# Autobot37/weatherforecastingtoolkit

Hardware: AMD Instinct MI355X
Metric: SEVIR 384x384 frames/sec (AE train step) (higher is better)
Workload: dtype f32; 1 GPU; experiments/ae_v2 conv AE (ae_64x8x8_lin.PosAwareAE_TF, img_size=384), 1x384x384 synthetic SEVIR frames, batch 32/GPU, fp32, fwd + L1 + bwd + AdamW + cosine-warmup LR; batch_per_gpu=32, global_batch=32, img_size=384, parallelism=dp1, params=215033281

## Files before the change

### include/wfae.h

```cpp
#ifndef WFAE_H
#define WFAE_H

#include <stddef.h>
#include <stdint.h>

#ifdef __cplusplus
extern "C" {
#endif

typedef void* wfae_stream_t;

typedef enum {
  WFAE_OK = 0,
  WFAE_ERR_BAD_SHAPE = -1,
  WFAE_ERR_NULL_POINTER = -2,
  WFAE_ERR_WORKSPACE = -3,
  WFAE_ERR_LAUNCH = -4,
  WFAE_ERR_UNSUPPORTED = -5
} wfae_status;

int wfae_version(void);
const char* wfae_last_error_string(void);
size_t wfae_workspace_bytes(int64_t max_weight_elems);

// ... 29 lines not shown
int wfae_c1r_stat_rows(int M, int K, int NB, int HW);
int wfae_c1r_fwd(const float* w, int64_t w_sm, int64_t w_sk, const float* x, const float* pro_scale, const float* pro_shift,
                 const float* res, float* y, int NB, int K, int M, int HW, double* stat_part, int64_t stat_capacity,
                 int* stat_rows, wfae_stream_t stream);
int wfae_c1r_bnred_supported(int M, int K, int HW);
int wfae_c1r_bnred(const float* w, int64_t w_sm, int64_t w_sk, const float* dt, const float* x, const float* bn_scale,
                   const float* bn_shift, const float* save_mean, const float* save_invstd, float* da, int NB, int K, int M, int HW,
                   double* part, int64_t part_capacity, int* part_rows, wfae_stream_t stream);
int wfae_bn_act_bwd_from_rows(const double* part, int rows, int C, float* dgamma, float* dbeta, int accumulate, void* ws,
                              size_t ws_bytes, wfae_stream_t stream);
int wfae_c1r_bndx(const float* w, int64_t w_sm, int64_t w_sk, const float* dt, const float* x, const float* gamma,
                  const float* bn_scale, const float* bn_shift, const float* save_mean, const float* save_invstd, const float* coef,
                  const float* res, float* dx, int NB, int K, int M, int HW, int training, wfae_stream_t stream);
int wfae_c1rb_supported(int M, int K, int HW);
int wfae_c1rb_stat_rows(int M, int K, int NB, int HW);
int wfae_c1rb_fwd(const float* w, int64_t w_sm, int64_t w_sk, const uint16_t* x, const float* pro_scale, const float* pro_shift,
                  const uint16_t* res, uint16_t* y, int NB, int K, int M, int HW, double* stat_part, int64_t stat_capacity,
                  int* stat_rows, wfae_stream_t stream);
int wfae_c1w_supported(int Cin, int Cout, int HW);
int wfae_c1w_bwd_weight(const float* dy, const float* x, const float* bn_scale, const float* bn_shift, float* dw, int NB, int Cin,
                        int Cout, int HW, int accumulate, void* ws, size_t ws_bytes, wfae_stream_t stream);
int wfae_c1w_bwd_weight_bf16(const uint16_t* dy, const uint16_t* x, const float* bn_scale, const float* bn_shift, float* dw, int NB,
                             int Cin, int Cout, int HW, int accumulate, void* ws, size_t ws_bytes, wfae_stream_t stream);
int wfae_set_c1wd(int on);
int wfae_get_c1wd(void);
int wfae_c1wd_supported(int C, int mid, int HW);
int wfae_c1wd_bwd(const float* dy, const float* t2, const float* bn_scale, const float* bn_shift, const float* w3, float* dw3,
                  float* da3, int NB, int C, int mid, int HW, int accumulate, void* ws, size_t ws_bytes, wfae_stream_t stream);
int wfae_set_c1ws(int on);
int wfae_get_c1ws(void);
int wfae_c1ws_supported(int C, int mid, int HW);
int wfae_c1ws_stat_rows(int C, int mid, int NB, int HW, size_t ws_bytes);
int wfae_c1ws_bwd(const float* x, const float* dt1, const float* bn_scale, const float* bn_shift, const float* save_mean,
                  const float* save_invstd, const float* w1, float* dw1, double* part, int64_t part_capacity, int* part_rows, int NB,
                  int C, int mid, int HW, int accumulate, void* ws, size_t ws_bytes, wfae_stream_t stream);
int wfae_linear_fwd(const float* x, const float* w, const float* bias, float* y, int B, int In,
                    int Out, void* ws, size_t ws_bytes, wfae_stream_t stream);
int wfae_linear_bwd_data(const float* dy, const float* w, float* dx, int B, int In, int Out,
                         wfae_stream_t stream);
int wfae_linear_bwd_weight(const float* dy, const float* x, float* dw, int B, int In, int Out,
                           int accumulate, wfae_stream_t stream);
int wfae_linear_bwd_data_splitk(const float* dy, const float* w, float* dx, int B, int In, int Out, void* ws,
                                size_t ws_bytes, wfae_stream_t stream);
int wfae_linear_bwd_weight_splitk(const float* dy, const float* x, float* dw, int B, int In, int Out, int accumulate,
                                  void* ws, size_t ws_bytes, wfae_stream_t stream);

int wfae_conv4x4s2_down(const float* hi, const float* w, float* lo, int NB, int Chi, int Clo,
                        int Hlo, int Wlo, wfae_stream_t stream);
int wfae_conv4x4s2_up(const float* lo, const float* w, float* hi, int NB, int Chi, int Clo, int Hlo,
                      int Wlo, void* ws, size_t ws_bytes, wfae_stream_t stream);
int wfae_conv4x4s2_wgrad(const float* lo, const float* hi, float* dw, int NB, int Chi, int Clo,
// ... 391 lines not shown
```

### weatherforecastingtoolkit_amd/csrc/c1w.hip

```cpp
#include "common.h"

using namespace wfae;

namespace {

typedef float f32x16 __attribute__((ext_vector_type(16)));
typedef __bf16 bf16x8 __attribute__((ext_vector_type(8)));
typedef unsigned u32x4 __attribute__((ext_vector_type(4)));
typedef unsigned u32x2 __attribute__((ext_vector_type(2)));

struct C1WP {
  const void* P;
  const void* Q;
  float* slab;
  const float* pro_scale;
  const float* pro_shift;
  int MP, MQ, HW;
  int cpi;
  int kc;
  int ptiles;
};

constexpr int WNT = 512, WBK = 32;

// ... 176 lines not shown
      __builtin_amdgcn_sched_barrier(0);
      read_frag(f0, cur ^ 1, 0);
      mfma_frag(f1);
      __builtin_amdgcn_sched_barrier(0);
    }
  }

  float* __restrict__ Cb = p.slab + (long)blockIdx.y * p.MP * p.MQ;
#pragma unroll
  for (int i = 0; i < TM; ++i)
#pragma unroll
    for (int j = 0; j < TN; ++j) {
      const int col = n0 + wn0 + 32 * j + r31;
#pragma unroll
      for (int q = 0; q < 16; ++q) {
        const int row = m0 + wm0 + 32 * i + (q & 3) + 8 * (q >> 2) + 4 * lh;
        if (row < p.MP && col < p.MQ) Cb[(long)row * p.MQ + col] = acc[i][j][q];
      }
    }
}

inline bool al16(const void* q) { return (reinterpret_cast<uintptr_t>(q) & 15) == 0; }

template <typename T, int PRO>
int launch_c1w(C1WP& p, int NB, hipStream_t st, const char* what) {
  const int tm = p.MP > 128 ? 2 : 1, tn = p.MQ > 64 ? 2 : 1;
  const int bm = 128 * tm, bn = 64 * tn;
  p.ptiles = cdiv(p.MP, bm);
  const int qtiles = cdiv(p.MQ, bn);
  const dim3 grid((unsigned)(p.ptiles * qtiles), (unsigned)(NB * p.cpi)), block(WNT);
  if (tm == 2 && tn == 2) hipLaunchKernelGGL((c1w_kernel<T, 2, 2, PRO>), grid, block, 0, st, p);
  else if (tm == 2) hipLaunchKernelGGL((c1w_kernel<T, 2, 1, PRO>), grid, block, 0, st, p);
  else if (tn == 2) hipLaunchKernelGGL((c1w_kernel<T, 1, 2, PRO>), grid, block, 0, st, p);
  else hipLaunchKernelGGL((c1w_kernel<T, 1, 1, PRO>), grid, block, 0, st, p);
  return check_launch(what);
}

inline bool c1w_shape_ok(int Cin, int Cout, int HW) {
  return HW % 32 == 0 && Cin % 32 == 0 && Cout % 32 == 0 && Cin >= 32 && Cout >= 32;
}

template <typename T>
int c1w_impl(const T* dy, const T* x, const float* bn_scale, const float* bn_shift, float* dw, int NB, int Cin, int Cout, int HW,
             int accumulate, void* ws, size_t ws_bytes, hipStream_t st, const char* what) {
  WFAE_REQUIRE(dy && x && dw && ws, WFAE_ERR_NULL_POINTER, "%s: null pointer", what);
  WFAE_REQUIRE(NB > 0 && Cin > 0 && Cout > 0 && HW > 0 && NB <= 65535, WFAE_ERR_BAD_SHAPE, "%s: bad shape", what);
  WFAE_REQUIRE(c1w_shape_ok(Cin, Cout, HW) && al16(dy) && al16(x), WFAE_ERR_UNSUPPORTED,
               "%s: needs HW %% 32 == 0, channel counts %% 32 == 0, 16-byte aligned tensors (Cin %d, Cout %d, HW %d)", what, Cin,
               Cout, HW);
  const bool x_is_p = Cin >= Cout;
  C1WP p = {};
  p.P = x_is_p ? (const void*)x : (const void*)dy;
  p.Q = x_is_p ? (const void*)dy : (const void*)x;
  p.MP = x_is_p ? Cin : Cout;
// ... 18 lines not shown

namespace wfae {

bool c1w_chunks(int MP, int MQ, int NB, int HW, size_t ws_bytes, int* cpi_out, int* kc_out) {
  const size_t slab = (size_t)MP * MQ * sizeof(float);
  const int tiles = cdiv(MP, MP > 128 ? 256 : 128) * cdiv(MQ, MQ > 64 ? 128 : 64);
  int cpi = cdiv(1024, (long)tiles * NB);
  const int max_cpi = HW / 256 > 0 ? HW / 256 : 1;
  if (cpi > max_cpi) cpi = max_cpi;
  if (cpi < 1) cpi = 1;
  while (cpi > 1 && (size_t)NB * cpi * slab > ws_bytes) --cpi;
  if ((size_t)NB * cpi * slab > ws_bytes) return false;
  *kc_out = cdiv(cdiv(HW, cpi), WBK) * WBK;
  *cpi_out = cdiv(HW, *kc_out);
  return true;
}

}

extern "C" {

int wfae_c1w_supported(int Cin, int Cout, int HW) { return c1w_shape_ok(Cin, Cout, HW) ? 1 : 0; }

int wfae_c1w_bwd_weight(const float* dy, const float* x, const float* bn_scale, const float* bn_shift, float* dw, int NB, int Cin,
                        int Cout, int HW, int accumulate, void* ws, size_t ws_bytes, wfae_stream_t stream) {
  WFAE_REQUIRE((bn_scale != nullptr) == (bn_shift != nullptr), WFAE_ERR_NULL_POINTER, "c1w_bwd_weight: scale / shift go together");
  return c1w_impl(dy, x, bn_scale, bn_shift, dw, NB, Cin, Cout, HW, accumulate, ws, ws_bytes, (hipStream_t)stream, "c1w_bwd_weight");
}

int wfae_c1w_bwd_weight_bf16(const uint16_t* dy, const uint16_t* x, const float* bn_scale, const float* bn_shift, float* dw, int NB,
                             int Cin, int Cout, int HW, int accumulate, void* ws, size_t ws_bytes, wfae_stream_t stream) {
  WFAE_REQUIRE((bn_scale != nullptr) == (bn_shift != nullptr), WFAE_ERR_NULL_POINTER, "c1w_bwd_weight_bf16: scale / shift go together");
  return c1w_impl(dy, x, bn_scale, bn_shift, dw, NB, Cin, Cout, HW, accumulate, ws, ws_bytes, (hipStream_t)stream,
                  "c1w_bwd_weight_bf16");
}

}
```

### weatherforecastingtoolkit_amd/csrc/c1wd.hip

```cpp
#include "common.h"
#include <atomic>
#include <stdlib.h>
#include <type_traits>

using namespace wfae;

namespace {

typedef float f32x4 __attribute__((ext_vector_type(4)));
typedef float f32x16 __attribute__((ext_vector_type(16)));
typedef __bf16 bf16x8 __attribute__((ext_vector_type(8)));
typedef short s16x4 __attribute__((ext_vector_type(4)));
typedef short s16x8 __attribute__((ext_vector_type(8)));
typedef unsigned u32x4 __attribute__((ext_vector_type(4)));
typedef unsigned u32x2 __attribute__((ext_vector_type(2)));

struct C1WDP {
  const float* dy;
  const float* t2;
  const float* w3;
  const float* pro_scale;
  const float* pro_shift;
  float* slab;
  float* da;
  int HW;
  int cpi;
  int kc;
};

constexpr int DNT = 512, DBK = 32;

__device__ __forceinline__ unsigned off_row(int r, int c) { return (unsigned)(r * 64 + ((c ^ ((r >> 2) & 3)) << 4)); }

__device__ __forceinline__ void split_pair(float a, float b, unsigned& h, unsigned& m, unsigned& l) {
  h = pack_bf16(a, b);
  const float ra = a - bf16_lo(h), rb = b - bf16_hi(h);
  m = pack_bf16(ra, rb);
  l = pack_bf16(ra - bf16_lo(m), rb - bf16_hi(m));
}

template <int C>
__global__ __launch_bounds__(DNT, C == 128 ? 4 : 2) void c1wd_kernel(C1WDP p) {
  constexpr int M = C / 4;
  constexpr int TM = C / 128;
  constexpr int WQ = M / 32;
  constexpr int NDW = 4 * WQ;
  constexpr bool BOTH = NDW == 8;
  constexpr int KCH = C / 32;
  constexpr int LPR = 8;
  constexpr int P_LD = C * LPR, Q_LD = M * LPR;
  constexpr int P_IT = P_LD / DNT;
  static_assert(P_LD % DNT == 0 && Q_LD <= DNT, "loader");
  constexpr int A_PLANE_B = C * 64, B_PLANE_B = M * 64;
  constexpr int A_STAGE_B = 3 * A_PLANE_B, STAGE_B = 3 * (A_PLANE_B + B_PLANE_B);
  __shared__ __attribute__((aligned(16))) unsigned char smem[2 * STAGE_B];
  const int t = threadIdx.x, lane = t & 63;
  const int wave = __builtin_amdgcn_readfirstlane(t >> 6);
  const int img = blockIdx.x / p.cpi, chunk = blockIdx.x - img * p.cpi;
  const int k_begin = chunk * p.kc;
  const int k_end = min(p.HW, k_begin + p.kc);
  const int nsteps = (k_end - k_begin) / DBK;
  const bool do_dw = BOTH || wave < NDW, do_da = BOTH || wave >= NDW;

  const float* Pb = p.dy + (long)img * C * p.HW + k_begin;
  const float* Qb = p.t2 + (long)img * M * p.HW + k_begin;
  const float* p_src[P_IT];
  unsigned p_dst[P_IT];
#pragma unroll
  for (int j = 0; j < P_IT; ++j) {
    const int idx = t + j * DNT, r = idx / LPR, e = idx % LPR;
    p_src[j] = Pb + (long)r * p.HW + e * 4;
    p_dst[j] = off_row(r, e >> 1) + (unsigned)((e & 1) * 8);
  }
  const bool q_on = Q_LD == DNT || t < Q_LD;
  const int q_r = q_on ? t / LPR : 0, q_e = t % LPR;
  const float* q_src = Qb + (long)q_r * p.HW + q_e * 4;
  const unsigned q_dst = off_row(q_r, q_e >> 1) + (unsigned)((q_e & 1) * 8);
  const float q_s = p.pro_scale[q_r], q_h = p.pro_shift[q_r];
  u32x4 rp[P_IT], rq;
  auto load_global = [&]() {
#pragma unroll
    for (int j = 0; j < P_IT; ++j) rp[j] = *reinterpret_cast<const u32x4*>(p_src[j]);
    if (q_on) rq = *reinterpret_cast<const u32x4*>(q_src);
  };
  auto advance = [&](bool more) {
#pragma unroll
    for (int j = 0; j < P_IT; ++j) p_src[j] += more ? DBK : 0;
    q_src += more ? DBK : 0;
  };
  auto put = [&](unsigned char* base, int plane_b, unsigned dst, u32x4 r, bool act, float s, float h) {
    const unsigned u0 = r[0], u1 = r[1], u2 = r[2], u3 = r[3];
    float v0 = __uint_as_float(u0), v1 = __uint_as_float(u1), v2 = __uint_as_float(u2), v3 = __uint_as_float(u3);
    if (act) {
      v0 = gelu_f(fmaf(v0, s, h)); v1 = gelu_f(fmaf(v1, s, h));
      v2 = gelu_f(fmaf(v2, s, h)); v3 = gelu_f(fmaf(v3, s, h));
    }
    unsigned h0, m0, l0, h1, m1, l1;
    split_pair(v0, v1, h0, m0, l0);
    split_pair(v2, v3, h1, m1, l1);
    *reinterpret_cast<u32x2*>(base + dst) = u32x2{h0, h1};
    *reinterpret_cast<u32x2*>(base + plane_b + dst) = u32x2{m0, m1};
    *reinterpret_cast<u32x2*>(base + 2 * plane_b + dst) = u32x2{l0, l1};
  };
  auto store_lds = [&](int buf) {
    unsigned char* s = smem + buf * STAGE_B;
#pragma unroll
    for (int j = 0; j < P_IT; ++j) put(s, A_PLANE_B, p_dst[j], rp[j], false, 0.f, 0.f);
    if (q_on) put(s + A_STAGE_B, B_PLANE_B, q_dst, rq, true, q_s, q_h);
  };

  const int wm0 = (BOTH ? (wave >> 1) : (wave & 3)) * (32 * TM), wn0 = BOTH ? (wave & 1) * 32 : 0;
  const int r31 = lane & 31, lh = lane >> 5;
  const unsigned a_rd = (unsigned)((wm0 + r31) * 64), b_rd = (unsigned)((wn0 + r31) * 64);
  const int a_x = (r31 >> 2) & 3;
  f32x16 acc[TM];
  struct Frag {
    bf16x8 a[TM][3], b[3];
  };
  auto read_frag = [&](Frag& f, int buf, int ks) {
    const unsigned char* s = smem + buf * STAGE_B;
    const unsigned a_c = (unsigned)(((2 * ks + lh) ^ a_x) << 4);
#pragma unroll
    for (int i = 0; i < TM; ++i)
#pragma unroll
      for (int pl = 0; pl < 3; ++pl)
        f.a[i][pl] = *reinterpret_cast<const bf16x8*>(s + pl * A_PLANE_B + a_rd + i * (32 * 64) + a_c);
#pragma unroll
    for (int pl = 0; pl < 3; ++pl) f.b[pl] = *reinterpret_cast<const bf16x8*>(s + A_STAGE_B + pl * B_PLANE_B + b_rd + a_c);
  };
  auto mfma_frag = [&](const Frag& f) {
#pragma unroll
// ... 15 lines not shown
  bf16x8 wa[KCH][3];
  auto load_weights = [&]() {
#pragma unroll
    for (int ch = 0; ch < KCH; ++ch) {
      const float* src = p.w3 + (long)(32 * ch + 8 * kg) * M + 16 * mt + n16;
      float v[8];
#pragma unroll
      for (int e = 0; e < 8; ++e) v[e] = src[e * M];
      u32x4 h, m, l;
#pragma unroll
      for (int e = 0; e < 4; ++e) {
        unsigned qh, qm, ql;
        split_pair(v[2 * e], v[2 * e + 1], qh, qm, ql);
        h[e] = qh; m[e] = qm; l[e] = ql;
      }
      wa[ch][0] = __builtin_bit_cast(bf16x8, h);
      wa[ch][1] = __builtin_bit_cast(bf16x8, m);
      wa[ch][2] = __builtin_bit_cast(bf16x8, l);
    }
  };
  unsigned tr_rd[2];
#pragma unroll
  for (int hf = 0; hf < 2; ++hf) tr_rd[hf] = off_row(8 * kg + 4 * hf + tq, 2 * pt + (tp >> 1)) + 8u * (unsigned)(tp & 1);
  float* const da_dst = p.da + ((long)img * M + 16 * mt + 4 * kg) * p.HW + k_begin + 16 * pt + n16;
  auto da_step = [&](int buf, int st) {
    const unsigned char* s = smem + buf * STAGE_B;
    constexpr int PA[6] = {2, 0, 1, 1, 0, 0}, PB[6] = {0, 2, 1, 0, 1, 0};
    f32x4 d = {0.f, 0.f, 0.f, 0.f};
#pragma unroll
    for (int ch = 0; ch < KCH; ++ch) {
      bf16x8 b[3];
#pragma unroll
      for (int pl = 0; pl < 3; ++pl) {
        s16x4 part[2];
#pragma unroll
        for (int hf = 0; hf < 2; ++hf)
          part[hf] = __builtin_amdgcn_ds_read_tr16_b64_v4i16(
              (s16x4 __attribute__((address_space(3)))*)(s + pl * A_PLANE_B + ch * (32 * 64) + tr_rd[hf]));
        b[pl] = __builtin_bit_cast(bf16x8, __builtin_shufflevector(part[0], part[1], 0, 1, 2, 3, 4, 5, 6, 7));
      }
#pragma unroll
      for (int pr = 0; pr < 6; ++pr) d = __builtin_amdgcn_mfma_f32_16x16x32_bf16(wa[ch][PA[pr]], b[PB[pr]], d, 0, 0, 0);
    }
    float* o = da_dst + 32 * st;
#pragma unroll
    for (int q = 0; q < 4; ++q) o[(long)q * p.HW] = d[q];
  };

  auto run = [&](auto dwc, auto dac) {
    constexpr bool DW = decltype(dwc)::value, DA = decltype(dac)::value;
    if constexpr (DW) {
#pragma unroll
      for (int i = 0; i < TM; ++i)
#pragma unroll
        for (int q = 0; q < 16; ++q) acc[i][q] = 0.f;
    }
    if constexpr (DA) load_weights();
    if (nsteps > 0) {
      Frag f0, f1;
      load_global();
      advance(nsteps > 1);
      store_lds(0);
      load_global();
      advance(nsteps > 2);
      __syncthreads();
      if constexpr (DW) read_frag(f0, 0, 0);
      for (int st = 0; st < nsteps; ++st) {
        const int cur = st & 1;
        if constexpr (DW) read_frag(f1, cur, 1);
        store_lds(cur ^ 1);
        load_global();
        advance(st + 3 < nsteps);
        if constexpr (DW) mfma_frag(f0);
        if constexpr (DA) da_step(cur, st);
        __builtin_amdgcn_sched_barrier(0);
        __syncthreads();
        __builtin_amdgcn_sched_barrier(0);
        if constexpr (DW) {
          read_frag(f0, cur ^ 1, 0);
          mfma_frag(f1);
        }
        __builtin_amdgcn_sched_barrier(0);
      }
    }
    if constexpr (DW) {
      float* __restrict__ Cb = p.slab + (long)blockIdx.x * C * M;
#pragma unroll
      for (int i = 0; i < TM; ++i)
#pragma unroll
        for (int q = 0; q < 16; ++q) {
          const int row = wm0 + 32 * i + (q & 3) + 8 * (q >> 2) + 4 * lh;
          Cb[(long)row * M + wn0 + r31] = acc[i][q];
        }
    }
  };
  if constexpr (BOTH) run(std::true_type{}, std::true_type{});
  else if (do_dw) run(std::true_type{}, std::false_type{});
  else run(std::false_type{}, std::true_type{});
}

std::atomic<int> g_c1wd{-1};
inline bool c1wd_on() {
  int v = g_c1wd.load(std::memory_order_relaxed);
  if (v < 0) {
    const char* e = getenv("WFAE_C1WD");
    v = (e && e[0] == '0') ? 0 : 1;
    g_c1wd.store(v, std::memory_order_relaxed);
  }
  return v == 1;
}

inline bool al16(const void* q) { return (reinterpret_cast<uintptr_t>(q) & 15) == 0; }

inline bool c1wd_shape_ok(int C, int mid, int HW) { return (C == 128 || C == 256) && mid * 4 == C && HW > 0 && HW % 64 == 0; }

}

extern "C" {

int wfae_set_c1wd(int on) {
  g_c1wd.store(on ? 1 : 0, std::memory_order_relaxed);
  return WFAE_OK;
}

int wfae_get_c1wd(void) { return c1wd_on() ? 1 : 0; }

int wfae_c1wd_supported(int C, int mid, int HW) {
  return (c1wd_on() && c1wd_shape_ok(C, mid, HW) && wfae::split_gemm_enabled()) ? 1 : 0;
}

int wfae_c1wd_bwd(const float* dy, const float* t2, const float* bn_scale, const float* bn_shift, const float* w3, float* dw3,
                  float* da3, int NB, int C, int mid, int HW, int accumulate, void* ws, size_t ws_bytes, wfae_stream_t stream) {
  WFAE_REQUIRE(dy && t2 && bn_scale && bn_shift && w3 && dw3 && da3 && ws, WFAE_ERR_NULL_POINTER, "c1wd_bwd: null pointer");
  WFAE_REQUIRE(NB > 0 && C > 0 && mid > 0 && HW > 0 && NB <= 65535 && (int64_t)NB * HW < (1ll << 31), WFAE_ERR_BAD_SHAPE,
               "c1wd_bwd: bad shape");
  WFAE_REQUIRE(c1wd_shape_ok(C, mid, HW), WFAE_ERR_UNSUPPORTED,
               "c1wd_bwd: serves C = 128 or 256 with mid = C / 4 and HW %% 64 == 0 (C %d, mid %d, HW %d)", C, mid, HW);
  WFAE_REQUIRE(c1wd_on() && wfae::split_gemm_enabled(), WFAE_ERR_UNSUPPORTED,
               "c1wd_bwd: needs fp32 precision with the split GEMMs on and wfae_set_c1wd(1)");
  WFAE_REQUIRE(al16(dy) && al16(t2), WFAE_ERR_UNSUPPORTED, "c1wd_bwd: dy and t2 must be 16-byte aligned");
  C1WDP p = {};
  p.dy = dy; p.t2 = t2; p.w3 = w3;
  p.pro_scale = bn_scale; p.pro_shift = bn_shift;
  p.slab = (float*)ws; p.da = da3;
  p.HW = HW;
  WFAE_REQUIRE(c1w_chunks(C, mid, NB, HW, ws_bytes, &p.cpi, &p.kc), WFAE_ERR_WORKSPACE, "c1wd_bwd: workspace %zu < %zu", ws_bytes,
               (size_t)NB * C * mid * sizeof(float));
  hipStream_t st = (hipStream_t)stream;
  const dim3 grid((unsigned)(NB * p.cpi)), block(DNT);
  if (C == 128) hipLaunchKernelGGL((c1wd_kernel<128>), grid, block, 0, st, p);
  else hipLaunchKernelGGL((c1wd_kernel<256>), grid, block, 0, st, p);
  const int rc = check_launch("c1wd_bwd");
  if (rc) return rc;
  return slab_reduce((const float*)ws, dw3, nullptr, (long)C * mid, mid, NB * p.cpi, accumulate, st, 0);
}

}
```

### weatherforecastingtoolkit_amd/functional.py

```python
from __future__ import annotations

import os

import torch
from torch.autograd import Function

from . import ops

BN_EPS = 1e-5


_overlap = False
_side = {}


STAT_FUSION = os.environ.get("WFAE_STAT_FUSION", "1") == "1"


FUSE_A1 = os.environ.get("WFAE_FUSE_A1", "1") == "1"
FUSE_A1_MAXC = 1 << 30
FUSE_A3 = os.environ.get("WFAE_FUSE_A3", "1") == "1"
FUSE_A3_MAXC = int(os.environ.get("WFAE_FUSE_A3_MAXC", "128"))
FUSE_A3_MAXC_C1R = max(FUSE_A3_MAXC, 256)

# ... 501 lines not shown
        t2 = _g3_fwd(a2, wg, groups)
        st3 = _bn_stats(t2, bn3, training)
        a3 = None if fused3 else ops.bn_act_fwd(t2, st3, 1)
        y, mod._out_stats = _c1(w3, W3p[0], False, *((t2, st3) if fused3 else (a3, None)), x, emit, r3)
        ctx.save_for_backward(x, _opt(a1), t1, a2, t2, _opt(a3), g1, w1, g2, wg, g3, w3,
                              st1.mean, st1.invstd, st1.scale, st1.shift,
                              st2.mean, st2.invstd, st2.scale, st2.shift,
                              st3.mean, st3.invstd, st3.scale, st3.shift,
                              _opt(W1p[1] if d1 == "c1b" else None), _opt(W3p[1] if d3 == "c1b" else None))
        ctx.training = training
        ctx.groups = groups
        ctx.betas = (b1, b2, b3)
        return y

    @staticmethod
    def backward(ctx, dy):
        (x, a1, t1, a2, t2, a3, g1, w1, g2, wg, g3, w3, *s) = ctx.saved_tensors
        st1, st2, st3 = _mk_stats(*s[0:4]), _mk_stats(*s[4:8]), _mk_stats(*s[8:12])
        W1t, W3t = s[12], s[13]
        tr = ctx.training
        dy = _c(dy)
        mid = w1.shape[0]
        dw3 = grad_buffer(w3)
        da3 = None
        if a3.numel() == 0:
            if ops.conv1x1_wd_route(dy.shape[1], mid, dy.shape[2] * dy.shape[3], _storage(dy)) == "c1wd":
                da3 = _on_main(lambda: ops.conv1x1_bwd_wd(dy, t2, st3, w3, dw3))
            if da3 is None:
                _wgrad(lambda: ops.conv1x1_bwd_weight_bnact(dy, t2, st3, dw3), dy, t2, st3.scale, st3.shift)
        else:
            _wgrad(lambda: ops.conv1x1_bwd_weight(dy, a3, dw3), dy, a3)
        dg3, db3 = grad_buffer(g3), grad_buffer(ctx.betas[2])
        if da3 is not None:
            dt2 = ops.bn_act_bwd(da3, t2, g3, st3, dg3, db3, None, 1, tr)
        else:
            dt2 = _dgrad_bn(dy, w3, W3t, t2, g3, st3, dg3, db3, None, tr)
        del da3
        dwg = grad_buffer(wg)
        _wgrad(lambda: _g3_wgrad(dt2, a2, dwg, ctx.groups), dt2, a2)
        da2 = _g3_dgrad(dt2, wg, mid, ctx.groups)
        del dt2
        dg2, db2 = grad_buffer(g2), grad_buffer(ctx.betas[1])
        dt1 = ops.bn_act_bwd(da2, t1, g2, st2, dg2, db2, None, 1, tr)
        del da2
        dw1 = grad_buffer(w1)
        rows1 = None
        if a1.numel() == 0:
            if ops.conv1x1_ws_route(x.shape[1], mid, x.shape[2] * x.shape[3], _storage(x)) == "c1ws":
                rows1 = _on_main(lambda: ops.conv1x1_bwd_ws(dt1, x, st1, w1, dw1))
            if rows1 is None:
                _wgrad(lambda: ops.conv1x1_bwd_weight_bnact(dt1, x, st1, dw1), dt1, x, st1.scale, st1.shift)
        else:
            _wgrad(lambda: ops.conv1x1_bwd_weight(dt1, a1, dw1), dt1, a1)
        dg1, db1 = grad_buffer(g1), grad_buffer(ctx.betas[0])
        dx = _dgrad_bn(dt1, w1, W1t, x, g1, st1, dg1, db1, dy, tr, rows1)
        return dx, dg1, db1, dw1, dg2, db2, dwg, dg3, db3, dw3, None, None
# ... 1064 lines not shown
```

### weatherforecastingtoolkit_amd/ops.py

```python
from __future__ import annotations

import ctypes
import math
import os

import torch

from . import _lib

_WS_DEFAULT = int(os.environ.get("WFAE_WORKSPACE_MB", "512")) << 20
_ws = {}


def _stream():
    return torch.cuda.current_stream().cuda_stream


_prof = None


def profile_start():
    global _prof
    _prof = {}

# ... 189 lines not shown
def set_c1r(on):
    global _C1R
    _C1R = bool(on)


def set_c1r_bnred(on):
    global _C1R_BNRED
    _C1R_BNRED = bool(on)


def set_c1r_bndx(on):
    global _C1R_BNDX
    _C1R_BNDX = bool(on)


def set_c1n(on):
    _lib.call("wfae_set_c1n", int(bool(on)))


def set_c1wd(on):
    _lib.call("wfae_set_c1wd", int(bool(on)))


def set_c1ws(on):
    _lib.call("wfae_set_c1ws", int(bool(on)))


def set_c1rb(on):
    global _C1RB
    _C1RB = bool(on)


def set_c1b(on):
    global _C1B
    _C1B = bool(on)


def set_c1w(on):
    global _C1W
    _C1W = bool(on)


def c1r_bndx_on():
    return _C1R_BNDX


def c1n_enabled():
    return bool(_lib.load().wfae_get_c1n())


def c1wd_enabled():
    return bool(_lib.load().wfae_get_c1wd())


def c1ws_enabled():
    return bool(_lib.load().wfae_get_c1ws())


def _precision():
    return _lib.load().wfae_get_matmul_precision()


def c1r_supported(m, k, hw):
    return _C1R and _SPLIT_GEMM and _precision() == 0 and bool(_lib.load().wfae_c1r_supported(int(m), int(k), int(hw)))


def c1r_bnred_supported(m, k, hw):
    return (_C1R and _C1R_BNRED and _SPLIT_GEMM and _precision() == 0
            and bool(_lib.load().wfae_c1r_bnred_supported(int(m), int(k), int(hw))))


def c1rb_supported(m, k, hw):
    return _C1RB and _precision() == 1 and bool(_lib.load().wfae_c1rb_supported(int(m), int(k), int(hw)))


# ... 142 lines not shown
        name, peak = "wfae_c1w_bwd_weight" + sfx, PEAK_BF16_MFMA / (1 if sfx else 6)
    elif sfx:
        name = "wfae_conv1x1_bwd_weight_bf16"
    else:
        name, pro = ("wfae_conv1x1_bwd_weight", ()) if st is None else ("wfae_conv1x1_bwd_weight_bnact", pro)
    ws = workspace()
    _call(name, 2 * n * cin * cout, es * n * (cin + cout) + 4 * cin * cout, _p(dy), _p(x), *pro, _p(dw), nb, cin, cout, h * wd,
          int(accumulate), ws.data_ptr(), ws.numel(), _stream(), peak=peak,
          label="wfae_conv1x1_bwd_weight" if st is None else "wfae_conv1x1_bwd_weight_bnact")
    return dw


def conv1x1_bwd_weight(dy, x, dw, accumulate=False):
    return _c1_wgrad(dy, x, None, dw, accumulate)


def conv1x1_bwd_weight_bnact(dy, x, st, dw, accumulate=False):
    return _c1_wgrad(dy, x, st, dw, accumulate)


C1WD_MIN_HW = 512


def conv1x1_wd_supported(c, mid, hw, storage="f32"):
    return (storage == "f32" and _SPLIT_GEMM and _precision() == 0 and bool(_lib.load().wfae_c1wd_supported(int(c), int(mid), int(hw)))
            and conv1x1_route("wgrad", c, mid, hw, "f32", True) == "c1w" and conv1x1_route("dgrad", mid, c, hw) == "c1r")


def conv1x1_wd_route(c, mid, hw, storage="f32"):
    return "c1wd" if hw >= C1WD_MIN_HW and conv1x1_wd_supported(c, mid, hw, storage) else "pair"


def conv1x1_bwd_wd(dy, t2, st, w3, dw3, accumulate=False):
    if st is None or dy.dtype != torch.float32 or t2.dtype != torch.float32:
        return None
    nb, c, h, wd = dy.shape
    mid, hw = t2.shape[1], h * wd
    if not conv1x1_wd_supported(c, mid, hw):
        return None
    _chk(dy, t2, w3, dw3)
    if tuple(t2.shape) != (nb, mid, h, wd) or w3.numel() != c * mid or dw3.numel() != c * mid:
        raise _lib.WfaeError("conv1x1_bwd_wd: dy (N, C, H, W), t2 (N, C/4, H, W), w3 and dw3 (C, C/4)")
    if (dy.data_ptr() | t2.data_ptr()) & 15:
        return None
    da = torch.empty_like(t2)
    n = nb * hw
    ws = workspace()
    _call("wfae_c1wd_bwd", 4 * n * c * mid, 4 * n * (c + 2 * mid) + 8 * c * mid, _p(dy), _p(t2), _p(st.scale), _p(st.shift), _p(w3),
          _p(dw3), _p(da), nb, c, mid, hw, int(accumulate), ws.data_ptr(), ws.numel(), _stream(), peak=PEAK_BF16_MFMA / 6,
          label="wfae_c1wd_bwd")
    return da


def conv1x1_ws_supported(c, mid, hw, storage="f32"):
    return (storage == "f32" and _SPLIT_GEMM and _precision() == 0 and bool(_lib.load().wfae_c1ws_supported(int(c), int(mid), int(hw)))
            and conv1x1_route("wgrad", mid, c, hw, "f32", True) == "c1w" and conv1x1_dgrad_bn_route(c, mid, hw, storage) == "bndx")


def conv1x1_ws_route(c, mid, hw, storage="f32"):
    return "c1ws" if hw >= C1WD_MIN_HW and conv1x1_ws_supported(c, mid, hw, storage) else "pair"


def conv1x1_bwd_ws(dt1, x, st, w1, dw1, accumulate=False):
    if st is None or dt1.dtype != torch.float32 or x.dtype != torch.float32:
        return None
    nb, c, h, wd = x.shape
    mid, hw = dt1.shape[1], h * wd
    if not conv1x1_ws_supported(c, mid, hw):
        return None
    _chk(dt1, x, w1, dw1)
# ... 2040 lines not shown
```

Baseline: 180.8 frames/s.

## Fuse BN3 backward statistics into c1wd kernel and add 128x256 c1w tile

Adds a stats variant of the fused conv1x1 wgrad/dgrad kernel that computes per-channel BN backward partial sums (gelu-grad times da, and times x-hat) while producing da3. The host then reduces those rows and runs only the dx part of BN backward, so da3 is no longer re-read just for the dgamma/dbeta reduction. It also adds a 128x256 tile option for the f32 c1w wgrad kernel with prologue when MQ>=256, aiming at better data reuse per block. Both are on by default through env-controlled flags. The costs are extra LDS, register pressure and a reordered pipeline in the fused kernel, which may lower occupancy.

New measurement: 182.2 frames/s (median of 6 runs). No clear change (+0.8%).

```diff
diff --git a/include/wfae.h b/include/wfae.h
--- a/include/wfae.h
+++ b/include/wfae.h
@@ -75,11 +75,22 @@
                         int Cout, int HW, int accumulate, void* ws, size_t ws_bytes, wfae_stream_t stream);
 int wfae_c1w_bwd_weight_bf16(const uint16_t* dy, const uint16_t* x, const float* bn_scale, const float* bn_shift, float* dw, int NB,
                              int Cin, int Cout, int HW, int accumulate, void* ws, size_t ws_bytes, wfae_stream_t stream);
+int wfae_set_c1w_tn4(int on);
+int wfae_get_c1w_tn4(void);
+int wfae_c1w_tile(int Cin, int Cout, int prologue, int* tile_p, int* tile_q);
+int wfae_c1w_slabs(int Cin, int Cout, int NB, int HW, size_t ws_bytes);
 int wfae_set_c1wd(int on);
 int wfae_get_c1wd(void);
 int wfae_c1wd_supported(int C, int mid, int HW);
 int wfae_c1wd_bwd(const float* dy, const float* t2, const float* bn_scale, const float* bn_shift, const float* w3, float* dw3,
                   float* da3, int NB, int C, int mid, int HW, int accumulate, void* ws, size_t ws_bytes, wfae_stream_t stream);
+int wfae_set_c1wd_bn3(int on);
+int wfae_get_c1wd_bn3(void);
+int wfae_c1wd_stat_rows(int C, int mid, int NB, int HW, size_t ws_bytes);
+int wfae_c1wd_bwd_stats(const float* dy, const float* t2, const float* bn_scale, const float* bn_shift, const float* save_mean,
+                        const float* save_invstd, const float* w3, float* dw3, float* da3, double* part, int64_t part_capacity,
+                        int* part_rows, int NB, int C, int mid, int HW, int accumulate, void* ws, size_t ws_bytes,
+                        wfae_stream_t stream);
 int wfae_set_c1ws(int on);
 int wfae_get_c1ws(void);
 int wfae_c1ws_supported(int C, int mid, int HW);
diff --git a/weatherforecastingtoolkit_amd/csrc/c1w.hip b/weatherforecastingtoolkit_amd/csrc/c1w.hip
--- a/weatherforecastingtoolkit_amd/csrc/c1w.hip
+++ b/weatherforecastingtoolkit_amd/csrc/c1w.hip
@@ -1,4 +1,6 @@
 #include "common.h"
+#include <atomic>
+#include <stdlib.h>
 
 using namespace wfae;
 
@@ -222,14 +224,37 @@
 
 inline bool al16(const void* q) { return (reinterpret_cast<uintptr_t>(q) & 15) == 0; }
 
+std::atomic<int> g_c1w_tn4{-1};
+inline bool c1w_tn4_on() {
+  int v = g_c1w_tn4.load(std::memory_order_relaxed);
+  if (v < 0) {
+    const char* e = getenv("WFAE_C1W_TN4");
+    v = (e && e[0] == '0') ? 0 : 1;
+    g_c1w_tn4.store(v, std::memory_order_relaxed);
+  }
+  return v == 1;
+}
+
+inline void c1w_tile(int MP, int MQ, bool f32, int pro, int* tm, int* tn) {
+  if (f32 && pro == 1 && MQ >= 256 && c1w_tn4_on()) {
+    *tm = 1; *tn = 4;
+    return;
+  }
+  *tm = MP > 128 ? 2 : 1;
+  *tn = MQ > 64 ? 2 : 1;
+}
+
 template <typename T, int PRO>
 int launch_c1w(C1WP& p, int NB, hipStream_t st, const char* what) {
-  const int tm = p.MP > 128 ? 2 : 1, tn = p.MQ > 64 ? 2 : 1;
-  const int bm = 128 * tm, bn = 64 * tn;
-  p.ptiles = cdiv(p.MP, bm);
-  const int qtiles = cdiv(p.MQ, bn);
+  int tm, tn;
+  c1w_tile(p.MP, p.MQ, sizeof(T) == 4, PRO, &tm, &tn);
+  p.ptiles = cdiv(p.MP, 128 * tm);
+  const int qtiles = cdiv(p.MQ, 64 * tn);
   const dim3 grid((unsigned)(p.ptiles * qtiles), (unsigned)(NB * p.cpi)), block(WNT);
-  if (tm == 2 && tn == 2) hipLaunchKernelGGL((c1w_kernel<T, 2, 2, PRO>), grid, block, 0, st, p);
+  if (tn == 4) {
+    if constexpr (sizeof(T) == 4 && PRO == 1) hipLaunchKernelGGL((c1w_kernel<T, 1, 4, PRO>), grid, block, 0, st, p);
+    else WFAE_REQUIRE(false, WFAE_ERR_UNSUPPORTED, "%s: no 128 x 256 tile for this form", what);
+  } else if (tm == 2 && tn == 2) hipLaunchKernelGGL((c1w_kernel<T, 2, 2, PRO>), grid, block, 0, st, p);
   else if (tm == 2) hipLaunchKernelGGL((c1w_kernel<T, 2, 1, PRO>), grid, block, 0, st, p);
   else if (tn == 2) hipLaunchKernelGGL((c1w_kernel<T, 1, 2, PRO>), grid, block, 0, st, p);
   else hipLaunchKernelGGL((c1w_kernel<T, 1, 1, PRO>), grid, block, 0, st, p);
@@ -294,6 +319,31 @@
 
 int wfae_c1w_supported(int Cin, int Cout, int HW) { return c1w_shape_ok(Cin, Cout, HW) ? 1 : 0; }
 
+int wfae_set_c1w_tn4(int on) {
+  g_c1w_tn4.store(on ? 1 : 0, std::memory_order_relaxed);
+  return WFAE_OK;
+}
+
+int wfae_get_c1w_tn4(void) { return c1w_tn4_on() ? 1 : 0; }
+
+int wfae_c1w_tile(int Cin, int Cout, int prologue, int* tile_p, int* tile_q) {
+  WFAE_REQUIRE(tile_p && tile_q, WFAE_ERR_NULL_POINTER, "c1w_tile: null pointer");
+  WFAE_REQUIRE(Cin > 0 && Cout > 0, WFAE_ERR_BAD_SHAPE, "c1w_tile: bad shape");
+  const bool x_is_p = Cin >= Cout;
+  int tm, tn;
+  c1w_tile(x_is_p ? Cin : Cout, x_is_p ? Cout : Cin, true, prologue ? (x_is_p ? 1 : 2) : 0, &tm, &tn);
+  *tile_p = 128 * tm;
+  *tile_q = 64 * tn;
+  return WFAE_OK;
+}
+
+int wfae_c1w_slabs(int Cin, int Cout, int NB, int HW, size_t ws_bytes) {
+  int cpi = 0, kc = 0;
+  if (!c1w_shape_ok(Cin, Cout, HW) || NB <= 0) return 0;
+  if (!c1w_chunks(Cin >= Cout ? Cin : Cout, Cin >= Cout ? Cout : Cin, NB, HW, ws_bytes, &cpi, &kc)) return 0;
+  return NB * cpi;
+}
+
 int wfae_c1w_bwd_weight(const float* dy, const float* x, const float* bn_scale, const float* bn_shift, float* dw, int NB, int Cin,
                         int Cout, int HW, int accumulate, void* ws, size_t ws_bytes, wfae_stream_t stream) {
   WFAE_REQUIRE((bn_scale != nullptr) == (bn_shift != nullptr), WFAE_ERR_NULL_POINTER, "c1w_bwd_weight: scale / shift go together");
diff --git a/weatherforecastingtoolkit_amd/csrc/c1wd.hip b/weatherforecastingtoolkit_amd/csrc/c1wd.hip
--- a/weatherforecastingtoolkit_amd/csrc/c1wd.hip
+++ b/weatherforecastingtoolkit_amd/csrc/c1wd.hip
@@ -23,12 +23,17 @@
   const float* pro_shift;
   float* slab;
   float* da;
+  const float* mean;
+  const float* invstd;
+  double* part0;
+  double* part1;
   int HW;
   int cpi;
   int kc;
 };
 
 constexpr int DNT = 512, DBK = 32;
+constexpr int T_LD = 20;
 
 __device__ __forceinline__ unsigned off_row(int r, int c) { return (unsigned)(r * 64 + ((c ^ ((r >> 2) & 3)) << 4)); }
 
@@ -39,7 +44,7 @@
   l = pack_bf16(ra - bf16_lo(m), rb - bf16_hi(m));
 }
 
-template <int C>
+template <int C, bool ST>
 __global__ __launch_bounds__(DNT, C == 128 ? 4 : 2) void c1wd_kernel(C1WDP p) {
   constexpr int M = C / 4;
   constexpr int TM = C / 128;
@@ -53,7 +58,9 @@
   static_assert(P_LD % DNT == 0 && Q_LD <= DNT, "loader");
   constexpr int A_PLANE_B = C * 64, B_PLANE_B = M * 64;
   constexpr int A_STAGE_B = 3 * A_PLANE_B, STAGE_B = 3 * (A_PLANE_B + B_PLANE_B);
-  __shared__ __attribute__((aligned(16))) unsigned char smem[2 * STAGE_B];
+  constexpr int T_WAVE_B = 16 * T_LD * 4;
+  constexpr int R_B = 8 * 16 * 2 * 8;
+  __shared__ __attribute__((aligned(16))) unsigned char smem[2 * STAGE_B + (ST ? 8 * T_WAVE_B + R_B : 0)];
   const int t = threadIdx.x, lane = t & 63;
   const int wave = __builtin_amdgcn_readfirstlane(t >> 6);
   const int img = blockIdx.x / p.cpi, chunk = blockIdx.x - img * p.cpi;
@@ -72,16 +79,23 @@
     p_src[j] = Pb + (long)r * p.HW + e * 4;
     p_dst[j] = off_row(r, e >> 1) + (unsigned)((e & 1) * 8);
   }
-  const bool q_on = Q_LD == DNT || t < Q_LD;
-  const int q_r = q_on ? t / LPR : 0, q_e = t % LPR;
+  const int q_tile = BOTH ? wave : (wave & 3);
+  const bool q_on = ST ? do_da : (Q_LD == DNT || t < Q_LD);
+  const int q_r = ST ? 16 * (q_tile >> 1) + (lane >> 2) : (q_on ? t / LPR : 0);
+  const int q_e = ST ? 4 * (q_tile & 1) + (lane & 3) : t % LPR;
   const float* q_src = Qb + (long)q_r * p.HW + q_e * 4;
   const unsigned q_dst = off_row(q_r, q_e >> 1) + (unsigned)((q_e & 1) * 8);
   const float q_s = p.pro_scale[q_r], q_h = p.pro_shift[q_r];
+  const float q_mu = ST ? p.mean[q_r] : 0.f, q_is = ST ? p.invstd[q_r] : 0.f;
   u32x4 rp[P_IT], rq;
-  auto load_global = [&]() {
+  float gp[4], xh[4];
+  double sum1 = 0.0, sum2 = 0.0;
+  auto load_global = [&](auto qc) {
 #pragma unroll
     for (int j = 0; j < P_IT; ++j) rp[j] = *reinterpret_cast<const u32x4*>(p_src[j]);
-    if (q_on) rq = *reinterpret_cast<const u32x4*>(q_src);
+    if constexpr (decltype(qc)::value) {
+      if (q_on) rq = *reinterpret_cast<const u32x4*>(q_src);
+    }
   };
   auto advance = [&](bool more) {
 #pragma unroll
@@ -102,11 +116,20 @@
     *reinterpret_cast<u32x2*>(base + plane_b + dst) = u32x2{m0, m1};
     *reinterpret_cast<u32x2*>(base + 2 * plane_b + dst) = u32x2{l0, l1};
   };
-  auto store_lds = [&](int buf) {
+  auto store_lds = [&](int buf, auto qc) {
     unsigned char* s = smem + buf * STAGE_B;
 #pragma unroll
     for (int j = 0; j < P_IT; ++j) put(s, A_PLANE_B, p_dst[j], rp[j], false, 0.f, 0.f);
-    if (q_on) put(s + A_STAGE_B, B_PLANE_B, q_dst, rq, true, q_s, q_h);
+    if constexpr (decltype(qc)::value) if (q_on) {
+      if constexpr (ST) {
+        const unsigned u0 = rq[0], u1 = rq[1], u2 = rq[2], u3 = rq[3];
+        const float x0 = __uint_as_float(u0), x1 = __uint_as_float(u1), x2 = __uint_as_float(u2), x3 = __uint_as_float(u3);
+        gp[0] = gelu_grad_f(fmaf(x0, q_s, q_h)); gp[1] = gelu_grad_f(fmaf(x1, q_s, q_h));
+        gp[2] = gelu_grad_f(fmaf(x2, q_s, q_h)); gp[3] = gelu_grad_f(fmaf(x3, q_s, q_h));
+        xh[0] = (x0 - q_mu) * q_is; xh[1] = (x1 - q_mu) * q_is; xh[2] = (x2 - q_mu) * q_is; xh[3] = (x3 - q_mu) * q_is;
+      }
+      put(s + A_STAGE_B, B_PLANE_B, q_dst, rq, true, q_s, q_h);
+    }
   };
 
   const int wm0 = (BOTH ? (wave >> 1) : (wave & 3)) * (32 * TM), wn0 = BOTH ? (wave & 1) * 32 : 0;
@@ -168,6 +191,9 @@
   unsigned tr_rd[2];
 #pragma unroll
   for (int hf = 0; hf < 2; ++hf) tr_rd[hf] = off_row(8 * kg + 4 * hf + tq, 2 * pt + (tp >> 1)) + 8u * (unsigned)(tp & 1);
+  unsigned char* const ttile = smem + 2 * STAGE_B + wave * T_WAVE_B;
+  float* const t_wr = reinterpret_cast<float*>(ttile) + (4 * kg) * T_LD + n16;
+  const f32x4* const t_rd = reinterpret_cast<const f32x4*>(ttile + ((lane >> 2) * T_LD + 4 * (lane & 3)) * 4);
   float* const da_dst = p.da + ((long)img * M + 16 * mt + 4 * kg) * p.HW + k_begin + 16 * pt + n16;
   auto da_step = [&](int buf, int st) {
     const unsigned char* s = smem + buf * STAGE_B;
@@ -191,10 +217,28 @@
     float* o = da_dst + 32 * st;
 #pragma unroll
     for (int q = 0; q < 4; ++q) o[(long)q * p.HW] = d[q];
+    if constexpr (ST) {
+#pragma unroll
+      for (int q = 0; q < 4; ++q) t_wr[q * T_LD] = d[q];
+    }
+  };
+  auto sums_step = [&]() {
+    __builtin_amdgcn_fence(__ATOMIC_RELEASE, "wavefront");
+    __builtin_amdgcn_wave_barrier();
+    __builtin_amdgcn_fence(__ATOMIC_ACQUIRE, "wavefront");
+    const f32x4 v = *t_rd;
+    const float d0 = v.x * gp[0], d1 = v.y * gp[1], d2 = v.z * gp[2], d3 = v.w * gp[3];
+    const float s1 = (d0 + d1) + (d2 + d3);
+    const float s2 = fmaf(d0, xh[0], d1 * xh[1]) + fmaf(d2, xh[2], d3 * xh[3]);
+    sum1 += (double)s1;
+    sum2 += (double)s2;
+    __builtin_amdgcn_fence(__ATOMIC_RELEASE, "wavefront");
+    __builtin_amdgcn_wave_barrier();
   };
 
   auto run = [&](auto dwc, auto dac) {
     constexpr bool DW = decltype(dwc)::value, DA = decltype(dac)::value;
+    constexpr std::bool_constant<!ST || DA> qc{};
     if constexpr (DW) {
 #pragma unroll
       for (int i = 0; i < TM; ++i)
@@ -204,29 +248,54 @@
     if constexpr (DA) load_weights();
     if (nsteps > 0) {
       Frag f0, f1;
-      load_global();
+      load_global(qc);
       advance(nsteps > 1);
-      store_lds(0);
-      load_global();
+      store_lds(0, qc);
+      load_global(qc);
       advance(nsteps > 2);
       __syncthreads();
-      if constexpr (DW) read_frag(f0, 0, 0);
-      for (int st = 0; st < nsteps; ++st) {
-        const int cur = st & 1;
-        if constexpr (DW) read_frag(f1, cur, 1);
-        store_lds(cur ^ 1);
-        load_global();
-        advance(st + 3 < nsteps);
-        if constexpr (DW) mfma_frag(f0);
-        if constexpr (DA) da_step(cur, st);
-        __builtin_amdgcn_sched_barrier(0);
-        __syncthreads();
-        __builtin_amdgcn_sched_barrier(0);
-        if constexpr (DW) {
-          read_frag(f0, cur ^ 1, 0);
+      if constexpr (ST && BOTH) {
+        for (int st = 0; st < nsteps; ++st) {
+          const int cur = st & 1;
+          da_step(cur, st);
+          sums_step();
+          __builtin_amdgcn_sched_barrier(0);
+          store_lds(cur ^ 1, qc);
+          load_global(qc);
+          advance(st + 3 < nsteps);
+          __builtin_amdgcn_sched_barrier(0);
+          read_frag(f0, cur, 0);
+          read_frag(f1, cur, 1);
+          mfma_frag(f0);
           mfma_frag(f1);
+          __builtin_amdgcn_sched_barrier(0);
+          __syncthreads();
+          __builtin_amdgcn_sched_barrier(0);
         }
-        __builtin_amdgcn_sched_barrier(0);
+      } else {
+        if constexpr (DW) read_frag(f0, 0, 0);
+        for (int st = 0; st < nsteps; ++st) {
+          const int cur = st & 1;
+          if constexpr (DW) read_frag(f1, cur, 1);
+          if constexpr (ST && DA) {
+            da_step(cur, st);
+            sums_step();
+            __builtin_amdgcn_sched_barrier(0);
+          }
+          store_lds(cur ^ 1, qc);
+          load_global(qc);
+          advance(st + 3 < nsteps);
+          if constexpr (DW) mfma_frag(f0);
+          if constexpr (DA && !ST) da_step(cur, st);
+          __builtin_amdgcn_sched_barrier(0);
+          __syncthreads();
+          __builtin_amdgcn_sched_barrier(0);
+          if constexpr (DW) {
+            read_frag(f0, cur ^ 1, 0);
+            mfma_frag(f1);
+          }
+          __builtin_amdgcn_sched_barrier(0);
+        }
       }
     }
     if constexpr (DW) {
@@ -243,6 +312,26 @@
   if constexpr (BOTH) run(std::true_type{}, std::true_type{});
   else if (do_dw) run(std::true_type{}, std::false_type{});
   else run(std::false_type{}, std::true_type{});
+
+  if constexpr (ST) {
+    double e1 = sum1, e2 = sum2;
+#pragma unroll
+    for (int o = 1; o < 4; o <<= 1) {
+      e1 += __shfl_xor(e1, o, 64);
+      e2 += __shfl_xor(e2, o, 64);
+    }
+    double* const red = reinterpret_cast<double*>(smem + 2 * STAGE_B + 8 * T_WAVE_B);
+    if (do_da && (q_tile & 1) && (lane & 3) == 0) {
+      red[(q_tile * 16 + (lane >> 2)) * 2 + 0] = e1;
+      red[(q_tile * 16 + (lane >> 2)) * 2 + 1] = e2;
+    }
+    __syncthreads();
+    if (do_da && !(q_tile & 1) && (lane & 3) == 0) {
+      const long at = (long)blockIdx.x * M + q_r;
+      p.part0[at] = e1 + red[((q_tile + 1) * 16 + (lane >> 2)) * 2 + 0];
+      p.part1[at] = e2 + red[((q_tile + 1) * 16 + (lane >> 2)) * 2 + 1];
+    }
+  }
 }
 
 std::atomic<int> g_c1wd{-1};
@@ -256,6 +345,17 @@
   return v == 1;
 }
 
+std::atomic<int> g_c1wd_bn3{-1};
+inline bool c1wd_bn3_on() {
+  int v = g_c1wd_bn3.load(std::memory_order_relaxed);
+  if (v < 0) {
+    const char* e = getenv("WFAE_C1WD_BN3");
+    v = (e && e[0] == '0') ? 0 : 1;
+    g_c1wd_bn3.store(v, std::memory_order_relaxed);
+  }
+  return v == 1;
+}
+
 inline bool al16(const void* q) { return (reinterpret_cast<uintptr_t>(q) & 15) == 0; }
 
 inline bool c1wd_shape_ok(int C, int mid, int HW) { return (C == 128 || C == 256) && mid * 4 == C && HW > 0 && HW % 64 == 0; }
@@ -275,8 +375,44 @@
   return (c1wd_on() && c1wd_shape_ok(C, mid, HW) && wfae::split_gemm_enabled()) ? 1 : 0;
 }
 
+static int c1wd_launch(const char* what, const float* dy, const float* t2, const float* bn_scale, const float* bn_shift,
+                       const float* save_mean, const float* save_invstd, const float* w3, float* dw3, float* da3, double* part,
+                       int64_t part_capacity, int* part_rows, int NB, int C, int mid, int HW, int accumulate, void* ws,
+                       size_t ws_bytes, wfae_stream_t stream);
+
 int wfae_c1wd_bwd(const float* dy, const float* t2, const float* bn_scale, const float* bn_shift, const float* w3, float* dw3,
                   float* da3, int NB, int C, int mid, int HW, int accumulate, void* ws, size_t ws_bytes, wfae_stream_t stream) {
+  return c1wd_launch("c1wd_bwd", dy, t2, bn_scale, bn_shift, nullptr, nullptr, w3, dw3, da3, nullptr, 0, nullptr, NB, C, mid, HW,
+                     accumulate, ws, ws_bytes, stream);
+}
+
+int wfae_set_c1wd_bn3(int on) {
+  g_c1wd_bn3.store(on ? 1 : 0, std::memory_order_relaxed);
+  return WFAE_OK;
+}
+
+int wfae_get_c1wd_bn3(void) { return c1wd_bn3_on() ? 1 : 0; }
+
+int wfae_c1wd_stat_rows(int C, int mid, int NB, int HW, size_t ws_bytes) {
+  int cpi = 0, kc = 0;
+  if (!c1wd_bn3_on() || !wfae_c1wd_supported(C, mid, HW) || NB <= 0 || !c1w_chunks(C, mid, NB, HW, ws_bytes, &cpi, &kc)) return 0;
+  return NB * cpi;
+}
+
+int wfae_c1wd_bwd_stats(const float* dy, const float* t2, const float* bn_scale, const float* bn_shift, const float* save_mean,
+                        const float* save_invstd, const float* w3, float* dw3, float* da3, double* part, int64_t part_capacity,
+                        int* part_rows, int NB, int C, int mid, int HW, int accumulate, void* ws, size_t ws_bytes,
+                        wfae_stream_t stream) {
+  WFAE_REQUIRE(save_mean && save_invstd && part && part_rows, WFAE_ERR_NULL_POINTER, "c1wd_bwd_stats: null pointer");
+  WFAE_REQUIRE(c1wd_bn3_on(), WFAE_ERR_UNSUPPORTED, "c1wd_bwd_stats: needs wfae_set_c1wd_bn3(1)");
+  return c1wd_launch("c1wd_bwd_stats", dy, t2, bn_scale, bn_shift, save_mean, save_invstd, w3, dw3, da3, part, part_capacity,
+                     part_rows, NB, C, mid, HW, accumulate, ws, ws_bytes, stream);
+}
+
+static int c1wd_launch(const char* what, const float* dy, const float* t2, const float* bn_scale, const float* bn_shift,
+                       const float* save_mean, const float* save_invstd, const float* w3, float* dw3, float* da3, double* part,
+                       int64_t part_capacity, int* part_rows, int NB, int C, int mid, int HW, int accumulate, void* ws,
+                       size_t ws_bytes, wfae_stream_t stream) {
   WFAE_REQUIRE(dy && t2 && bn_scale && bn_shift && w3 && dw3 && da3 && ws, WFAE_ERR_NULL_POINTER, "c1wd_bwd: null pointer");
   WFAE_REQUIRE(NB > 0 && C > 0 && mid > 0 && HW > 0 && NB <= 65535 && (int64_t)NB * HW < (1ll << 31), WFAE_ERR_BAD_SHAPE,
                "c1wd_bwd: bad shape");
@@ -293,10 +429,20 @@
   WFAE_REQUIRE(c1w_chunks(C, mid, NB, HW, ws_bytes, &p.cpi, &p.kc), WFAE_ERR_WORKSPACE, "c1wd_bwd: workspace %zu < %zu", ws_bytes,
                (size_t)NB * C * mid * sizeof(float));
   hipStream_t st = (hipStream_t)stream;
-  const dim3 grid((unsigned)(NB * p.cpi)), block(DNT);
-  if (C == 128) hipLaunchKernelGGL((c1wd_kernel<128>), grid, block, 0, st, p);
-  else hipLaunchKernelGGL((c1wd_kernel<256>), grid, block, 0, st, p);
-  const int rc = check_launch("c1wd_bwd");
+  const int rows = NB * p.cpi;
+  const dim3 grid((unsigned)rows), block(DNT);
+  if (part) {
+    WFAE_REQUIRE(part_capacity >= 2 * (int64_t)rows * mid, WFAE_ERR_WORKSPACE, "c1wd_bwd_stats: part holds %lld doubles, needs %lld",
+                 (long long)part_capacity, (long long)(2 * (int64_t)rows * mid));
+    *part_rows = rows;
+    p.mean = save_mean; p.invstd = save_invstd;
+    p.part0 = part;
+    p.part1 = part + (long)rows * mid;
+    if (C == 128) hipLaunchKernelGGL((c1wd_kernel<128, true>), grid, block, 0, st, p);
+    else hipLaunchKernelGGL((c1wd_kernel<256, true>), grid, block, 0, st, p);
+  } else if (C == 128) hipLaunchKernelGGL((c1wd_kernel<128, false>), grid, block, 0, st, p);
+  else hipLaunchKernelGGL((c1wd_kernel<256, false>), grid, block, 0, st, p);
+  const int rc = check_launch(what);
   if (rc) return rc;
   return slab_reduce((const float*)ws, dw3, nullptr, (long)C * mid, mid, NB * p.cpi, accumulate, st, 0);
 }
diff --git a/weatherforecastingtoolkit_amd/functional.py b/weatherforecastingtoolkit_amd/functional.py
--- a/weatherforecastingtoolkit_amd/functional.py
+++ b/weatherforecastingtoolkit_amd/functional.py
@@ -547,16 +547,24 @@
         dy = _c(dy)
         mid = w1.shape[0]
         dw3 = grad_buffer(w3)
-        da3 = None
+        da3 = rows3 = None
         if a3.numel() == 0:
-            if ops.conv1x1_wd_route(dy.shape[1], mid, dy.shape[2] * dy.shape[3], _storage(dy)) == "c1wd":
+            how = ops.conv1x1_wd_bn3_route(dy.shape[1], mid, dy.shape[2] * dy.shape[3], _storage(dy))
+            if how == "rows":
+                r = _on_main(lambda: ops.conv1x1_bwd_wd(dy, t2, st3, w3, dw3, stats=True))
+                if r is not None:
+                    da3, rows3 = r
+            elif how == "c1wd":
                 da3 = _on_main(lambda: ops.conv1x1_bwd_wd(dy, t2, st3, w3, dw3))
             if da3 is None:
                 _wgrad(lambda: ops.conv1x1_bwd_weight_bnact(dy, t2, st3, dw3), dy, t2, st3.scale, st3.shift)
         else:
             _wgrad(lambda: ops.conv1x1_bwd_weight(dy, a3, dw3), dy, a3)
         dg3, db3 = grad_buffer(g3), grad_buffer(ctx.betas[2])
-        if da3 is not None:
+        if rows3 is not None:
+            ops.bn_act_bwd_from_rows(rows3, mid, dg3, db3)
+            dt2 = ops.bn_act_bwd_dx(da3, t2, g3, st3, None, 1, tr)
+        elif da3 is not None:
             dt2 = ops.bn_act_bwd(da3, t2, g3, st3, dg3, db3, None, 1, tr)
         else:
             dt2 = _dgrad_bn(dy, w3, W3t, t2, g3, st3, dg3, db3, None, tr)
diff --git a/weatherforecastingtoolkit_amd/ops.py b/weatherforecastingtoolkit_amd/ops.py
--- a/weatherforecastingtoolkit_amd/ops.py
+++ b/weatherforecastingtoolkit_amd/ops.py
@@ -235,6 +235,14 @@
     _lib.call("wfae_set_c1wd", int(bool(on)))
 
 
+def set_c1w_tn4(on):
+    _lib.call("wfae_set_c1w_tn4", int(bool(on)))
+
+
+def set_c1wd_bn3(on):
+    _lib.call("wfae_set_c1wd_bn3", int(bool(on)))
+
+
 def set_c1ws(on):
     _lib.call("wfae_set_c1ws", int(bool(on)))
 
@@ -264,6 +272,21 @@
 
 def c1wd_enabled():
     return bool(_lib.load().wfae_get_c1wd())
+
+
+def c1w_tn4_enabled():
+    return bool(_lib.load().wfae_get_c1w_tn4())
+
+
+def c1wd_bn3_enabled():
+    return bool(_lib.load().wfae_get_c1wd_bn3())
+
+
+def c1w_tile(cin, cout, prologue):
+    a, b = ctypes.c_int(0), ctypes.c_int(0)
+    _lib.call("wfae_c1w_tile", int(cin), int(cout), int(bool(prologue)), ctypes.cast(ctypes.pointer(a), ctypes.c_void_p),
+              ctypes.cast(ctypes.pointer(b), ctypes.c_void_p))
+    return a.value, b.value
 
 
 def c1ws_enabled():
@@ -452,6 +475,14 @@
 C1WD_MIN_HW = 512
 
 
+C1WD_BN3_MIN_HW = 192 * 192
+
+
+def conv1x1_wd_bn3_route(c, mid, hw, storage="f32"):
+    r = conv1x1_wd_route(c, mid, hw, storage)
+    return "rows" if r == "c1wd" and hw >= C1WD_BN3_MIN_HW and c1wd_bn3_enabled() else r
+
+
 def conv1x1_wd_supported(c, mid, hw, storage="f32"):
     return (storage == "f32" and _SPLIT_GEMM and _precision() == 0 and bool(_lib.load().wfae_c1wd_supported(int(c), int(mid), int(hw)))
             and conv1x1_route("wgrad", c, mid, hw, "f32", True) == "c1w" and conv1x1_route("dgrad", mid, c, hw) == "c1r")
@@ -461,7 +492,7 @@
     return "c1wd" if hw >= C1WD_MIN_HW and conv1x1_wd_supported(c, mid, hw, storage) else "pair"
 
 
-def conv1x1_bwd_wd(dy, t2, st, w3, dw3, accumulate=False):
+def conv1x1_bwd_wd(dy, t2, st, w3, dw3, accumulate=False, stats=False):
     if st is None or dy.dtype != torch.float32 or t2.dtype != torch.float32:
         return None
     nb, c, h, wd = dy.shape
@@ -476,6 +507,15 @@
     da = torch.empty_like(t2)
     n = nb * hw
     ws = workspace()
+    if stats:
+        cap = 2 * int(_lib.load().wfae_c1wd_stat_rows(c, mid, nb, hw, ws.numel())) * mid
+        if cap <= 0:
+            return conv1x1_bwd_wd(dy, t2, st, w3, dw3, accumulate), None
+        part, rows, out = _rows_out(cap, dy.device)
+        _call("wfae_c1wd_bwd_stats", 4 * n * c * mid, 4 * n * (c + 2 * mid) + 8 * c * mid, _p(dy), _p(t2), _p(st.scale), _p(st.shift),
+              _p(st.mean), _p(st.invstd), _p(w3), _p(dw3), _p(da), *out, nb, c, mid, hw, int(accumulate), ws.data_ptr(), ws.numel(),
+              _stream(), peak=PEAK_BF16_MFMA / 6, label="wfae_c1wd_bwd")
+        return da, StatRows(part[:2 * rows.value * mid], rows.value)
     _call("wfae_c1wd_bwd", 4 * n * c * mid, 4 * n * (c + 2 * mid) + 8 * c * mid, _p(dy), _p(t2), _p(st.scale), _p(st.shift), _p(w3),
           _p(dw3), _p(da), nb, c, mid, hw, int(accumulate), ws.data_ptr(), ws.numel(), _stream(), peak=PEAK_BF16_MFMA / 6,
           label="wfae_c1wd_bwd")
```
